# togheppi/pytorch-super-resolution-model-collection

Measured on AMD Instinct MI355X. Metric: ESPCN x4 LR->HR images/sec (infer), higher is better.
Workload: dtype f32 storage/accumulate; fp32-faithful products on the fp16 matrix cores: operands scaled by exact powers of two, split into two fp16 planes, 3 MFMAs per product (f16x3, ~3e-7 rms vs fp64, like fp32 MFMA); 1 GPU; c2: ESPCN x4 inference, 256x256 LR, batch 64 per GPU, fp32, random-init N(0,0.02); parallelism=replicas x1 (no collective)

## Files before the change

### pytorch_super_resolution_model_collection_amd/csrc/conv_pair.hip

```cpp
#include "conv_bfw.h"

namespace srk {

namespace {

constexpr int PR_TH = 8, PR_TW = 16, PR_HW = 18;
constexpr int PR_NSLOTPIX = 6 * PR_HW, PR_NPIXP = PR_NSLOTPIX + 2;
constexpr int PR_NKEEP = 2 * PR_HW, PR_KP = PR_NKEEP + 2;
constexpr int PR_XR = 14, PR_XC = 23, PR_XP = 24;
constexpr int PR_NSLOT = 3, PR_NKBUF = 3;
constexpr int PR_WL2 = 9 * 2 * 256;
constexpr int PR_HBUF = 4 * PR_NPIXP;
constexpr int PR_KBUF = 2 * 4 * PR_KP;
constexpr int PR_PLANE = PR_NSLOT * PR_HBUF + PR_NKBUF * PR_KBUF;
constexpr int PR_XBUF = 2 * PR_XR * PR_XP;
constexpr unsigned PR_AMAX_CAP = 1u << 14;
constexpr int PR_ARRIVE = 1, PR_DEPART = 2;
constexpr int PR_XLD = 24;
constexpr int PR_W1P = 2 * 2 * 4 * 2 * 64;
constexpr int PR_W1P_FLOATS = 144;
constexpr size_t PR_W1P_BYTES = (size_t)PR_W1P * 16 + PR_W1P_FLOATS * 4;
constexpr size_t PR_LDS = (size_t)PR_WL2 * 16 + (size_t)2 * PR_PLANE * 16 + (size_t)2 * PR_XBUF * 8 + 64;
static_assert(PR_LDS <= 160 * 1024, "k_espcn_pair: LDS");

__device__ unsigned g_pair_timeouts = 0;
__device__ unsigned g_pair_scans = 0;

typedef unsigned v4u_t __attribute__((ext_vector_type(4)));

struct PairParams {
  const float* x;
  const uint4* w1p;
  const float* b1;
  const uint4* wq2;
  const float* w2_descale;
  const float* b2;
  float* y;
  float* x_amax;
  float* y_amax;
  size_t xn;
  int amax_mode;
  int N, H, W, OH, OW, tiles_y, img_tiles, ntiles;
  unsigned x_img_bytes, y_bytes;
};

__device__ __forceinline__ float pr_slice_absmax(const float* __restrict__ x, size_t lo, size_t hi, size_t n, bool tail,
                                                 int t, int nt) {
  const f32x4* x4 = reinterpret_cast<const f32x4*>(x);
  float m = 0.f;
  for (size_t base = lo; base < hi; base += (size_t)nt * PR_XLD) {
    f32x4 v[PR_XLD];
#pragma unroll
    for (int k = 0; k < PR_XLD; ++k) {
      const size_t e = base + (size_t)t + (size_t)k * nt;
      v[k] = x4[e < hi ? e : hi - 1];
    }
#pragma unroll
    for (int k = 0; k < PR_XLD; ++k) m = abs_max4(m, v[k]);
  }
  if (tail) {
    const size_t e = (n & ~(size_t)3) + (size_t)t;
    if (t < 3 && e < n) m = fmaxf(m, fabsf(x[e]));
  }
  return m;
}

__global__ __launch_bounds__(128) void k_espcn_pair_prep(const float* __restrict__ w1, const float* __restrict__ b1,
                                                         uint4* __restrict__ out) {
  const int lane = threadIdx.x & 63, c1 = threadIdx.x >> 6;
  const int j = lane & 15, kq = lane >> 4;
  float wsum = 0.f, wmax = 0.f;
  {
    const float* wc = w1 + lane * 75;
    for (int i = 0; i < 75; ++i) {
      const float a = fabsf(wc[i]);
      wsum += a;
      wmax = fmaxf(wmax, a);
    }
  }
  const float wm = wave_max(wmax);
  const float sw1 = exp2i(amax_scale_exp(wm));
#pragma unroll
  for (int nf = 0; nf < 2; ++nf) {
    const int co = c1 * 32 + nf * 16 + j;
#pragma unroll
    for (int ks = 0; ks < 4; ++ks) {
      const int q = 4 * ks + kq, dy = q / 3, dx0 = 2 * (q - 3 * (q / 3));
      float f[8];
#pragma unroll
      for (int e = 0; e < 8; ++e) {
        const int dx = dx0 + (e >> 2), ci = e & 3;
        const bool on = q < 15 && ci < 3 && dx < 5;
        f[e] = on ? w1[((co * 3 + (on ? ci : 0)) * 5 + (on ? dy : 0)) * 5 + (on ? dx : 0)] : 0.f;
      }
      uint4 pl[2];
      split8h(f, sw1, pl);
      out[(((c1 * 2 + nf) * 4 + ks) * 2 + 0) * 64 + lane] = pl[0];
      out[(((c1 * 2 + nf) * 4 + ks) * 2 + 1) * 64 + lane] = pl[1];
    }
  }
  if (c1 == 0) {
    float* t = reinterpret_cast<float*>(out + PR_W1P);
    t[lane] = wsum;
    t[64 + lane] = fabsf(b1[lane]);
    if (lane == 0) t[128] = wm;
  }
}

__global__ __launch_bounds__(512, 1) void k_espcn_pair(PairParams B) {
  extern __shared__ __attribute__((aligned(16))) uint4 smem4[];
  uint4* wl2 = smem4;
  uint4* ring = smem4 + PR_WL2;
  uint4* keep = ring + PR_NSLOT * PR_HBUF;
  uint2* xin_all = reinterpret_cast<uint2*>(ring + 2 * PR_PLANE);
  lds_cnt_t* cnt = (lds_cnt_t*)(xin_all + 2 * PR_XBUF);
  const int tid = threadIdx.x, lane = tid & 63, wave = tid >> 6;
  const int grp = wave >> 2, gw = wave & 3, lt = tid & 255;
  const int j = lane & 15, kq = lane >> 4;
  uint2* xin = xin_all + grp * PR_XBUF;

  const float* w1t = reinterpret_cast<const float*>(B.w1p + PR_W1P);
  const int nblk = gridDim.x;
  float xmax = 0.f;
  if (tid < 14) cnt[tid] = 0u;
  if (B.amax_mode) {
    float* red = reinterpret_cast<float*>(xin_all);
    const size_t n4 = B.xn >> 2;
    const float m = wave_max(pr_slice_absmax(B.x, (size_t)blockIdx.x * n4 / nblk, (size_t)(blockIdx.x + 1) * n4 / nblk, B.xn,
                                             blockIdx.x == 0, tid, 512));
    if (lane == 0) red[wave] = m;
    __syncthreads();
    if (tid == 0) {
      float b = red[0];
#pragma unroll
      for (int i = 1; i < 8; ++i) b = fmaxf(b, red[i]);
      const unsigned was = atomicMax(reinterpret_cast<unsigned*>(B.x_amax + (blockIdx.x & 15) * 16), __float_as_uint(b));
      asm volatile("s_waitcnt vmcnt(0)" ::"v"(was) : "memory");
      __hip_atomic_fetch_add(reinterpret_cast<unsigned*>(B.x_amax) + PR_ARRIVE, 1u, __ATOMIC_RELAXED, __HIP_MEMORY_SCOPE_AGENT);
    }
  } else {
    xmax = amax_read(B.x_amax);
  }

  {
    static_assert(PR_WL2 == 9 * 512, "k_espcn_pair: filter copy");
    v4u_t wv[9];
#pragma unroll
    for (int i = 0; i < 9; ++i) wv[i] = *reinterpret_cast<const v4u_t*>(B.wq2 + tid + 512 * i);
#pragma unroll
    for (int i = 0; i < 9; ++i) *reinterpret_cast<v4u_t*>(wl2 + tid + 512 * i) = wv[i];
  }

  const int c1 = gw >> 1, mh = gw & 1;
  const int mhu = __builtin_amdgcn_readfirstlane(mh), rhu = __builtin_amdgcn_readfirstlane(gw >> 1);
  uint4 w1f[2][4][2];
#pragma unroll
  for (int nf = 0; nf < 2; ++nf)
#pragma unroll
    for (int ks = 0; ks < 4; ++ks)
#pragma unroll
      for (int pl = 0; pl < 2; ++pl) w1f[nf][ks][pl] = B.w1p[(((c1 * 2 + nf) * 4 + ks) * 2 + pl) * 64 + lane];
  const float wsum = w1t[lane], babs = w1t[64 + lane];
  int koff[4], mpix[5], moff[5], tpix[2], toff[2];
#pragma unroll
  for (int ks = 0; ks < 4; ++ks) {
    const int q = (4 * ks + kq) < 15 ? 4 * ks + kq : 14;
    koff[ks] = (q / 3) * PR_XP + 2 * (q - 3 * (q / 3));
  }
#pragma unroll
  for (int m = 0; m < 5; ++m) {
    mpix[m] = 16 * (m < 4 ? 4 * mh + m : 8) + j;
    const int p = PR_NKEEP + mpix[m];
    moff[m] = (p / PR_HW) * PR_XP + p % PR_HW;
  }
#pragma unroll
  for (int m = 0; m < 2; ++m) {
    tpix[m] = 16 * (2 * mh + m) + j;
    const int p = tpix[m] < PR_NKEEP ? tpix[m] : PR_NKEEP - 1;
    toff[m] = (p / PR_HW) * PR_XP + p % PR_HW;
  }
  const int wr_slot = (kq >> 1) * PR_NPIXP * 16 + (kq & 1) * 8, wr_keep = (c1 * 4 + (kq >> 1)) * PR_KP * 16 + (kq & 1) * 8;

  const int rh = gw >> 1, nf2 = gw & 1;
  const int pj = j < 4 ? 2 * j : (j < 12 ? 2 * j - 7 : 2 * j - 16);
  const int lane_b = (4 * rh - 2) * PR_HW + pj + kq * PR_NPIXP;
  const int lane_k = pj + kq * PR_KP;
  const int lane_a = kq * 32 + nf2 * 16 + j;
  float b2v[4];
#pragma unroll
  for (int e = 0; e < 4; ++e) b2v[e] = B.b2[nf2 * 16 + 4 * kq + e];

  const int xcd = blockIdx.x & 7;
  int first, count;
  {
    const int lb = xcd * (nblk >> 3) + (xcd < (nblk & 7) ? xcd : (nblk & 7)) + (blockIdx.x >> 3);
    const int per = B.ntiles / nblk, rem = B.ntiles - per * nblk;
    first = lb * per + (lb < rem ? lb : rem);
    count = per + (lb < rem ? 1 : 0);
  }
  count = __builtin_amdgcn_readfirstlane(count);

  const __amdgpu_buffer_rsrc_t yr = buffer_rsrc(B.y, B.y_bytes);
  const unsigned HW_ = (unsigned)(B.H * B.W);
  float xv[2][3];
  auto xload = [&](int i) {
    const bool valid = i < count;
    const int t = first + (valid ? i : 0);
    const int n = t / B.img_tiles, rem = t - n * B.img_tiles;
    const int tx = rem / B.tiles_y, ty = rem - tx * B.tiles_y;
    const __amdgpu_buffer_rsrc_t xr = buffer_rsrc(B.x + (size_t)n * 3 * HW_, B.x_img_bytes);
#pragma unroll
    for (int s = 0; s < 2; ++s) {
      const int q = lt + 256 * s, qy = q / PR_XC, qx = q - qy * PR_XC;
      const bool ok = valid && q < PR_XR * PR_XC;
      const unsigned o = ok ? 4u * (unsigned)((ty * PR_TH + qy) * B.W + tx * PR_TW + qx) : 0x80000000u;
#pragma unroll
      for (int c = 0; c < 3; ++c)
        xv[s][c] = __builtin_bit_cast(float, __builtin_amdgcn_raw_buffer_load_b32(xr, (int)(o + (ok ? 4u * c * HW_ : 0u)), 0, 0));
    }
  };
  auto l1_frags = [&](auto nm, const int* off, f32x4 (*a)[2]) {
    constexpr int NM = decltype(nm)::value;
#pragma unroll
    for (int m = 0; m < NM; ++m) a[m][0] = a[m][1] = (f32x4){0.f, 0.f, 0.f, 0.f};
#pragma unroll
    for (int ks = 0; ks < 4; ++ks) {
#pragma unroll
      for (int m = 0; m < NM; ++m) {
        const int pa = off[m] + koff[ks];
        const uint2 h0 = xin[pa], h1 = xin[pa + 1];
        const uint2 l0 = xin[PR_XR * PR_XP + pa], l1 = xin[PR_XR * PR_XP + pa + 1];
        const uint4 xh = make_uint4(h0.x, h0.y, h1.x, h1.y), xm = make_uint4(l0.x, l0.y, l1.x, l1.y);
#pragma unroll
        for (int nf = 0; nf < 2; ++nf) {
          a[m][nf] = mfma16h(w1f[nf][ks][0], xm, a[m][nf]);
          a[m][nf] = mfma16h(w1f[nf][ks][1], xh, a[m][nf]);
          a[m][nf] = mfma16h(w1f[nf][ks][0], xh, a[m][nf]);
        }
      }
    }
  };
  bool dead = false;
  float amax = 0.f;
  xload(grp);
  if (B.amax_mode && wave == 0) {
    unsigned* ctr = reinterpret_cast<unsigned*>(B.x_amax);
    bool late = B.amax_mode == 2;
    if (!late) {
      unsigned spins = 0;
      while ((int)((unsigned)__builtin_amdgcn_readfirstlane((int)__hip_atomic_load(ctr + PR_ARRIVE, __ATOMIC_RELAXED,
                                                                                   __HIP_MEMORY_SCOPE_AGENT)) -
                   (unsigned)nblk) < 0) {
        __builtin_amdgcn_s_sleep(16);
        if (++spins > PR_AMAX_CAP) {
          late = true;
          break;
        }
      }
    }
    asm volatile("" ::: "memory");
    const float sv = wave_max(__hip_atomic_load(B.x_amax + (lane & 15) * 16, __ATOMIC_RELAXED, __HIP_MEMORY_SCOPE_AGENT));
    if (lane == 0) {
      cnt[14] = __float_as_uint(sv);
      cnt[15] = late ? 1u : 0u;
      const unsigned d = __hip_atomic_fetch_add(ctr + PR_DEPART, 1u, __ATOMIC_RELAXED, __HIP_MEMORY_SCOPE_AGENT);
      if (d + 1u == (unsigned)nblk) {
        __hip_atomic_store(ctr + PR_ARRIVE, 0u, __ATOMIC_RELAXED, __HIP_MEMORY_SCOPE_AGENT);
        __hip_atomic_store(ctr + PR_DEPART, 0u, __ATOMIC_RELAXED, __HIP_MEMORY_SCOPE_AGENT);
      }
    }
  }
  __syncthreads();
  if (B.amax_mode) {
    xmax = __uint_as_float(lds_cnt_peek(cnt + 14));
    if (lds_cnt_peek(cnt + 15)) {
      float* red = reinterpret_cast<float*>(xin_all);
      const float m = wave_max(pr_slice_absmax(B.x, 0, B.xn >> 2, B.xn, true, tid, 512));
      if (lane == 0) red[wave] = m;
      __syncthreads();
#pragma unroll
      for (int i = 0; i < 8; ++i) xmax = fmaxf(xmax, red[i]);
      xmax = __uint_as_float((unsigned)__builtin_amdgcn_readfirstlane((int)__float_as_uint(xmax)));
      __syncthreads();
      if (tid == 0) atomicAdd(&g_pair_scans, 1u);
    }
  }
  const int kx = amax_scale_exp(xmax);
  const float bnd = wave_max(fabsf(babs) + wsum * xmax);
  const int kw1 = amax_scale_exp(w1t[128]);
  const int km = amax_scale_exp(bnd);
  const float sx1 = exp2i(kx), sxm = exp2i(km);
  const float dsc1 = exp2i(-kx) * exp2i(-kw1);
  const float dsc2 = exp2i(-km) * B.w2_descale[0];

  unsigned own = 0;
  unsigned kseq = 0;
  int typrev = 0;
  for (int i = grp; i < count; i += 2, ++own) {
    const int t = first + i;
    const int n = t / B.img_tiles, rem = t - n * B.img_tiles;
    const int tx = rem / B.tiles_y, ty = rem - tx * B.tiles_y;
    const bool fresh = i == 0 || ty == 0;
    const bool hand = i + 1 < count && ty + 1 < B.tiles_y;
    kseq = i == grp ? (grp == 0 ? 1u : 2u + (ty == 0 ? 1u : 0u))
                    : kseq + 2u + (typrev + 1 == B.tiles_y ? 1u : 0u) + (ty == 0 ? 1u : 0u);
    typrev = ty;
    const unsigned kb = kseq % PR_NKBUF, ku = kseq / PR_NKBUF, tb = (kseq - 1u) % PR_NKBUF, tu = (kseq - 1u) / PR_NKBUF;
#pragma unroll
    for (int s = 0; s < 2; ++s) {
      const int q = lt + 256 * s;
      if (q < PR_XR * PR_XC) {
        const int qy = q / PR_XC, qx = q - qy * PR_XC;
        unsigned h01, m01, h2, m2;
        split2h(xv[s][0], xv[s][1], sx1, h01, m01);
        split2h(xv[s][2], 0.f, sx1, h2, m2);
        xin[qy * PR_XP + qx] = make_uint2(h01, h2);
        xin[PR_XR * PR_XP + qy * PR_XP + qx] = make_uint2(m01, m2);
      }
    }
    lds_cnt_signal(cnt + 6 + grp);
    xload(i + 2);
    lds_cnt_wait(cnt + 6 + grp, 4u * (own + 1), dead);

    float b1v[2][4];
#pragma unroll
    for (int nf = 0; nf < 2; ++nf)
#pragma unroll
      for (int e = 0; e < 4; ++e) b1v[nf][e] = B.b1[c1 * 32 + nf * 16 + 4 * kq + e];
    auto l1_store = [&](const f32x4 (&a)[2], unsigned char* base, int pix, int pitch) {
#pragma unroll
      for (int nf = 0; nf < 2; ++nf) {
        float v[4];
#pragma unroll
        for (int e = 0; e < 4; ++e) v[e] = fmaxf(__builtin_fmaf(a[nf][e], dsc1, b1v[nf][e]), 0.f);
        unsigned h01, m01, h23, m23;
        split2h(v[0], v[1], sxm, h01, m01);
        split2h(v[2], v[3], sxm, h23, m23);
        *reinterpret_cast<uint2*>(base + ((2 * nf) * pitch + pix) * 16) = make_uint2(h01, h23);
        *reinterpret_cast<uint2*>(base + (PR_PLANE + (2 * nf) * pitch + pix) * 16) = make_uint2(m01, m23);
      }
    };
    auto l1_tile = [&](auto nm) {
      constexpr int NM = decltype(nm)::value;
      f32x4 a1[NM][2];
      l1_frags(nm, moff, a1);
      const unsigned st = 2u * (unsigned)i + c1, slot = st % PR_NSLOT, use = st / PR_NSLOT;
      unsigned char* hb = reinterpret_cast<unsigned char*>(ring + slot * PR_HBUF) + wr_slot;
      lds_cnt_wait(cnt + 3 + slot, 4u * use, dead);
#pragma unroll
      for (int m = 0; m < NM; ++m)
        if (mpix[m] < PR_NSLOTPIX) l1_store(a1[m], hb, mpix[m], PR_NPIXP);
      lds_cnt_signal(cnt + slot);
      unsigned char* kp = reinterpret_cast<unsigned char*>(keep + kb * PR_KBUF) + wr_keep;
      lds_cnt_wait(cnt + 11 + kb, 8u * ku, dead);
#pragma unroll
      for (int m = 2; m < NM; ++m)
        if (mpix[m] >= PR_NSLOTPIX) l1_store(a1[m], kp, mpix[m] - PR_NSLOTPIX, PR_KP);
      lds_cnt_signal(cnt + 8 + kb);
    };
    const int vr = B.OH - ty * PR_TH;
    if (mhu == 1 && vr <= 3) {
      const unsigned st = 2u * (unsigned)i + c1, slot = st % PR_NSLOT, use = st / PR_NSLOT;
      lds_cnt_wait(cnt + 3 + slot, 4u * use, dead);
      lds_cnt_signal(cnt + slot);
      lds_cnt_wait(cnt + 11 + kb, 8u * ku, dead);
      lds_cnt_signal(cnt + 8 + kb);
    } else if (mh == (int)(own & 1)) {
      l1_tile(std::integral_constant<int, 5>{});
    } else {
      l1_tile(std::integral_constant<int, 4>{});
    }
    if (fresh) {
      f32x4 at[2][2];
      l1_frags(std::integral_constant<int, 2>{}, toff, at);
      unsigned char* kp = reinterpret_cast<unsigned char*>(keep + tb * PR_KBUF) + wr_keep;
      lds_cnt_wait(cnt + 11 + tb, 8u * tu, dead);
#pragma unroll
      for (int m = 0; m < 2; ++m)
        if (tpix[m] < PR_NKEEP) l1_store(at[m], kp, tpix[m], PR_KP);
      lds_cnt_signal(cnt + 8 + tb);
    }

    lds_cnt_wait(cnt + 8 + (rh == 0 ? tb : kb), 4u * ((rh == 0 ? tu : ku) + 1u), dead);
    if (rhu == 1 && vr <= 4) {
#pragma unroll
      for (int cc = 0; cc < 2; ++cc) {
        const unsigned st = 2u * (unsigned)i + cc, slot = st % PR_NSLOT, use = st / PR_NSLOT;
        lds_cnt_wait(cnt + slot, 2u * (use + 1), dead);
        lds_cnt_signal(cnt + 3 + slot);
      }
      lds_cnt_signal(cnt + 11 + tb, fresh ? 2u : 1u);
      lds_cnt_signal(cnt + 11 + kb, hand ? 1u : 2u);
    } else {
      f32x4 acc[4];
#pragma unroll
      for (int r = 0; r < 4; ++r) acc[r] = (f32x4){0.f, 0.f, 0.f, 0.f};
#pragma unroll
      for (int cc = 0; cc < 2; ++cc) {
        const unsigned st = 2u * (unsigned)i + cc, slot = st % PR_NSLOT, use = st / PR_NSLOT;
        lds_cnt_wait(cnt + slot, 2u * (use + 1), dead);
        const uint4* hb = ring + slot * PR_HBUF + lane_b;
        const uint4* kr = keep + (rh == 0 ? tb : kb) * PR_KBUF + cc * 4 * PR_KP + lane_k - (rh == 0 ? 0 : 4 * PR_HW);
        const uint4* pa = rh == 0 ? kr : hb;
        const uint4* pc = rh == 0 ? hb : kr;
#pragma unroll
        for (int v = 0; v < 3; ++v) {
          uint4 fa[3][2];
#pragma unroll
          for (int u = 0; u < 3; ++u) {
            fa[u][0] = wl2[((u * 3 + v) * 2 + cc) * 256 + lane_a];
            fa[u][1] = wl2[((u * 3 + v) * 2 + cc) * 256 + 128 + lane_a];
          }
#pragma unroll
          for (int R = 0; R < 6; ++R) {
            const uint4* px = R < 2 ? pa : (R < 4 ? hb : pc);
            const uint4 xh = px[R * PR_HW + v], xm = px[R * PR_HW + v + PR_PLANE];
#pragma unroll
            for (int u = 0; u < 3; ++u) {
              const int r = R - u;
              if (r >= 0 && r < 4) {
                acc[r] = mfma16h(fa[u][0], xm, acc[r]);
                acc[r] = mfma16h(fa[u][1], xh, acc[r]);
                acc[r] = mfma16h(fa[u][0], xh, acc[r]);
              }
            }
          }
        }
        lds_cnt_signal(cnt + 3 + slot);
      }
      lds_cnt_signal(cnt + 11 + tb, fresh ? 2u : 1u);
      lds_cnt_signal(cnt + 11 + kb, hand ? 1u : 2u);
      const int oc = tx * PR_TW + pj;
#pragma unroll
      for (int r = 0; r < 4; ++r) {
        const int orow = ty * PR_TH + 4 * rh + r;
        const bool ok = oc < B.OW && orow < B.OH;
        f32x4 v;
#pragma unroll
        for (int e = 0; e < 4; ++e) v[e] = fmaxf(__builtin_fmaf(acc[r][e], dsc2, b2v[e]), 0.f);
        if (ok) amax = fmaxf(amax, fmaxf(fmaxf(v[0], v[1]), fmaxf(v[2], v[3])));
        const unsigned o = ok ? 4u * (unsigned)(((n * B.OH + orow) * B.OW + oc) * 32 + nf2 * 16 + 4 * kq) : 0x80000000u;
        __builtin_amdgcn_raw_buffer_store_b128(__builtin_bit_cast(v4u_t, v), yr, (int)o, 0, 0);
      }
    }
  }
  if (B.y_amax) amax_commit(B.y_amax, amax, blockIdx.x + wave, amax_peek(B.y_amax, blockIdx.x + wave));
  if (dead && lane == 0) atomicAdd(&g_pair_timeouts, 1u);
}

}

int espcn_pair_launch(int N, int H, int W, const float* x, const void* w1p, const float* b1, const void* wp2,
                      const float* b2, float* y, float* x_amax, int amax_mode, float* y_amax, bool force, hipStream_t s) {
  if (N < 1 || H < 7 || W < 7 || !x_amax) return -1;
  const int OH = H - 6, OW = W - 6;
  const int tiles_y = (OH + PR_TH - 1) / PR_TH, tiles_x = (OW + PR_TW - 1) / PR_TW;
  const long ntiles = (long)N * tiles_y * tiles_x;
  const size_t x_img = (size_t)3 * H * W * 4, y_bytes = (size_t)N * OH * OW * 32 * 4;
  if (ntiles >= (1L << 29) || x_img >= (1ull << 31) || y_bytes >= (1ull << 31)) return -1;
  if (!force) {
    if ((double)OH * OW < 0.85 * (double)tiles_y * tiles_x * (PR_TH * PR_TW)) return -1;
    if (ntiles < 4L * kNumCU) return -1;
  }
  const size_t elems = (size_t)9 * 64 * 32;
  const char* prepared = reinterpret_cast<const char*>(wp2) + bf3_prepared_offset(elems);
  const char* fsec = prepared + f16_section_offset(64, 32, 9);
  PairParams B{};
  B.x = x; B.w1p = reinterpret_cast<const uint4*>(w1p); B.b1 = b1; B.b2 = b2; B.y = y; B.x_amax = x_amax; B.y_amax = y_amax;
  B.xn = (size_t)N * 3 * H * W;
  B.amax_mode = amax_mode;
  B.wq2 = reinterpret_cast<const uint4*>(fsec);
  B.w2_descale = reinterpret_cast<const float*>(fsec + bf3_main_bytes(64, 32, 9));
  B.N = N; B.H = H; B.W = W; B.OH = OH; B.OW = OW; B.tiles_y = tiles_y; B.img_tiles = tiles_x * tiles_y;
  B.ntiles = (int)ntiles;
  B.x_img_bytes = (unsigned)x_img;
  B.y_bytes = (unsigned)y_bytes;
  int grid = kNumCU;
  if (grid > ntiles) grid = (int)ntiles;
  note_amax_written(y_amax != nullptr);
  note_kernel("k_espcn_pair");
  launch_lds<&k_espcn_pair>(dim3(grid), dim3(512), PR_LDS, s, B);
  return check_launch("espcn_pair");
}

int pair_ring_timeouts(int reset) {
  unsigned v = 0;
  if (hipMemcpyFromSymbol(&v, HIP_SYMBOL(g_pair_timeouts), sizeof(v)) != hipSuccess) {
    (void)hipGetLastError();
    return -1;
  }
  if (reset && v) {
    const unsigned z = 0;
    (void)hipMemcpyToSymbol(HIP_SYMBOL(g_pair_timeouts), &z, sizeof(z));
  }
  return (int)v;
}

int pair_scans(int reset) {
  unsigned v = 0;
  if (hipMemcpyFromSymbol(&v, HIP_SYMBOL(g_pair_scans), sizeof(v)) != hipSuccess) {
    (void)hipGetLastError();
    return -1;
  }
  if (reset && v) {
    const unsigned z = 0;
    (void)hipMemcpyToSymbol(HIP_SYMBOL(g_pair_scans), &z, sizeof(z));
  }
  return (int)v;
}

int espcn_pair_prepare(const float* w1, const float* b1, void* out, hipStream_t s) {
  hipLaunchKernelGGL(k_espcn_pair_prep, dim3(1), dim3(128), 0, s, w1, b1, reinterpret_cast<uint4*>(out));
  return check_launch("espcn_pair_prepare");
}
size_t espcn_pair_prepared_bytes() { return PR_W1P_BYTES; }

}

extern "C" size_t srk_espcn_pair_prepared_bytes(void) { return srk::espcn_pair_prepared_bytes(); }

extern "C" int srk_espcn_pair_prepare(const float* w1, const float* b1, void* w1_prepared, void* stream) {
  SRK_REQUIRE(w1 && b1 && w1_prepared, "espcn_pair_prepare: null pointer");
  SRK_REQUIRE((uintptr_t)w1_prepared % 16 == 0, "espcn_pair_prepare: w1_prepared must be 16-byte aligned");
  return srk::espcn_pair_prepare(w1, b1, w1_prepared, (hipStream_t)stream);
}

extern "C" int srk_espcn_pair_scans(int reset) { return srk::pair_scans(reset); }

extern "C" int srk_espcn_pair_forward(int N, int H, int W, const float* x, const void* w1_prepared, const float* b1,
                                      const float* w2_packed_fwd, const float* b2, float* y, float* x_amax,
                                      int x_amax_compute, float* y_amax, int force, void* stream) {
  if (!x || !w1_prepared || !b1 || !w2_packed_fwd || !b2 || !y || !x_amax) return SRK_ERR_UNSUPPORTED;
  if (((uintptr_t)x | (uintptr_t)y | (uintptr_t)w1_prepared) % 16 != 0) return SRK_ERR_UNSUPPORTED;
  const int mode = x_amax_compute ? ((force & 2) ? 2 : 1) : 0;
  const int rc = srk::espcn_pair_launch(N, H, W, x, w1_prepared, b1, w2_packed_fwd, b2, y, x_amax, mode, y_amax,
                                        (force & 1) != 0, (hipStream_t)stream);
  return rc == -1 ? SRK_ERR_UNSUPPORTED : rc;
}
```

Measured before the change: 74320 images/s.

## Repack conv1 input and weights to fold fp16 split products into fewer MFMAs

Reorganizes the first conv layer's K dimension so that the hi/lo fp16 planes of the input and weights are packed into the same 8-element K slot. One MFMA per k-group then computes the cross terms, replacing three MFMAs over four k-steps with one MFMA over eight k-steps. The input tile in LDS becomes a 16-byte-per-pixel interleaved layout plus a transposed row buffer for the leftover taps, and pixels within the MFMA tile are permuted. This adds zero-initialisation of the input buffers and more complex addressing, and it risks changing the numerical equivalence of the split-fp16 scheme.

```diff
diff --git a/pytorch_super_resolution_model_collection_amd/csrc/conv_pair.hip b/pytorch_super_resolution_model_collection_amd/csrc/conv_pair.hip
--- a/pytorch_super_resolution_model_collection_amd/csrc/conv_pair.hip
+++ b/pytorch_super_resolution_model_collection_amd/csrc/conv_pair.hip
@@ -13,14 +13,17 @@
 constexpr int PR_HBUF = 4 * PR_NPIXP;
 constexpr int PR_KBUF = 2 * 4 * PR_KP;
 constexpr int PR_PLANE = PR_NSLOT * PR_HBUF + PR_NKBUF * PR_KBUF;
-constexpr int PR_XBUF = 2 * PR_XR * PR_XP;
+constexpr int PR_XPQ = PR_XR * PR_XP * 16;
+constexpr int PR_XT = PR_XPQ + 32;
+constexpr int PR_XBUF = PR_XT + PR_XR * PR_XP * 8;
+constexpr unsigned long long PR_FPIX = 0xfdb9eca875316420ull;
 constexpr unsigned PR_AMAX_CAP = 1u << 14;
 constexpr int PR_ARRIVE = 1, PR_DEPART = 2;
 constexpr int PR_XLD = 24;
-constexpr int PR_W1P = 2 * 2 * 4 * 2 * 64;
+constexpr int PR_W1P = 2 * 2 * 8 * 64;
 constexpr int PR_W1P_FLOATS = 144;
 constexpr size_t PR_W1P_BYTES = (size_t)PR_W1P * 16 + PR_W1P_FLOATS * 4;
-constexpr size_t PR_LDS = (size_t)PR_WL2 * 16 + (size_t)2 * PR_PLANE * 16 + (size_t)2 * PR_XBUF * 8 + 64;
+constexpr size_t PR_LDS = (size_t)PR_WL2 * 16 + (size_t)2 * PR_PLANE * 16 + (size_t)2 * PR_XBUF + 64;
 static_assert(PR_LDS <= 160 * 1024, "k_espcn_pair: LDS");
 
 __device__ unsigned g_pair_timeouts = 0;
@@ -65,6 +68,17 @@
   return m;
 }
 
+enum { PR_KTAP, PR_KROW, PR_KNONE };
+struct PrKGroup {
+  int kind, dy, dx;
+};
+__device__ __forceinline__ constexpr PrKGroup pr_kgroup(int ks, int kq) {
+  if (ks < 5) return {PR_KTAP, ks, kq};
+  if (ks == 5) return {PR_KTAP, (kq >> 1) + 2 * (kq & 1), 4};
+  if (ks == 6) return kq == 0 ? PrKGroup{PR_KTAP, 4, 4} : (kq == 1 ? PrKGroup{PR_KNONE, 0, 0} : PrKGroup{PR_KROW, 2 * kq - 4, 0});
+  return kq == 3 ? PrKGroup{PR_KNONE, 0, 0} : PrKGroup{PR_KROW, kq == 2 ? 4 : 2 * kq + 1, 0};
+}
+
 __global__ __launch_bounds__(128) void k_espcn_pair_prep(const float* __restrict__ w1, const float* __restrict__ b1,
                                                          uint4* __restrict__ out) {
   const int lane = threadIdx.x & 63, c1 = threadIdx.x >> 6;
@@ -84,19 +98,19 @@
   for (int nf = 0; nf < 2; ++nf) {
     const int co = c1 * 32 + nf * 16 + j;
 #pragma unroll
-    for (int ks = 0; ks < 4; ++ks) {
-      const int q = 4 * ks + kq, dy = q / 3, dx0 = 2 * (q - 3 * (q / 3));
+    for (int ks = 0; ks < 8; ++ks) {
+      const PrKGroup g = pr_kgroup(ks, kq);
       float f[8];
 #pragma unroll
       for (int e = 0; e < 8; ++e) {
-        const int dx = dx0 + (e >> 2), ci = e & 3;
-        const bool on = q < 15 && ci < 3 && dx < 5;
-        f[e] = on ? w1[((co * 3 + (on ? ci : 0)) * 5 + (on ? dy : 0)) * 5 + (on ? dx : 0)] : 0.f;
+        const bool tap = g.kind == PR_KTAP;
+        const bool on = tap || (g.kind == PR_KROW && e < 5);
+        const int ci = tap ? (e < 6 ? e % 3 : e - 6) : 2, dx = tap ? g.dx : (e < 5 ? e : 0);
+        f[e] = on ? w1[((co * 3 + ci) * 5 + g.dy) * 5 + dx] : 0.f;
       }
       uint4 pl[2];
       split8h(f, sw1, pl);
-      out[(((c1 * 2 + nf) * 4 + ks) * 2 + 0) * 64 + lane] = pl[0];
-      out[(((c1 * 2 + nf) * 4 + ks) * 2 + 1) * 64 + lane] = pl[1];
+      out[((c1 * 2 + nf) * 8 + ks) * 64 + lane] = g.kind == PR_KTAP ? make_uint4(pl[0].x, pl[0].y, pl[0].z, pl[1].w) : pl[1];
     }
   }
   if (c1 == 0) {
@@ -112,12 +126,12 @@
   uint4* wl2 = smem4;
   uint4* ring = smem4 + PR_WL2;
   uint4* keep = ring + PR_NSLOT * PR_HBUF;
-  uint2* xin_all = reinterpret_cast<uint2*>(ring + 2 * PR_PLANE);
+  unsigned char* xin_all = reinterpret_cast<unsigned char*>(ring + 2 * PR_PLANE);
   lds_cnt_t* cnt = (lds_cnt_t*)(xin_all + 2 * PR_XBUF);
   const int tid = threadIdx.x, lane = tid & 63, wave = tid >> 6;
   const int grp = wave >> 2, gw = wave & 3, lt = tid & 255;
   const int j = lane & 15, kq = lane >> 4;
-  uint2* xin = xin_all + grp * PR_XBUF;
+  unsigned char* xin = xin_all + grp * PR_XBUF;
 
   const float* w1t = reinterpret_cast<const float*>(B.w1p + PR_W1P);
   const int nblk = gridDim.x;
@@ -153,31 +167,35 @@
 
   const int c1 = gw >> 1, mh = gw & 1;
   const int mhu = __builtin_amdgcn_readfirstlane(mh), rhu = __builtin_amdgcn_readfirstlane(gw >> 1);
-  uint4 w1f[2][4][2];
+  uint4 w1f[2][8];
 #pragma unroll
   for (int nf = 0; nf < 2; ++nf)
 #pragma unroll
-    for (int ks = 0; ks < 4; ++ks)
-#pragma unroll
-      for (int pl = 0; pl < 2; ++pl) w1f[nf][ks][pl] = B.w1p[(((c1 * 2 + nf) * 4 + ks) * 2 + pl) * 64 + lane];
+    for (int ks = 0; ks < 8; ++ks) w1f[nf][ks] = B.w1p[((c1 * 2 + nf) * 8 + ks) * 64 + lane];
   const float wsum = w1t[lane], babs = w1t[64 + lane];
-  int koff[4], mpix[5], moff[5], tpix[2], toff[2];
-#pragma unroll
-  for (int ks = 0; ks < 4; ++ks) {
-    const int q = (4 * ks + kq) < 15 ? 4 * ks + kq : 14;
-    koff[ks] = (q / 3) * PR_XP + 2 * (q - 3 * (q / 3));
-  }
+  const int jp = (int)((PR_FPIX >> (4 * j)) & 15);
+  int mpix[5], moff[5], tpix[2], toff[2];
 #pragma unroll
   for (int m = 0; m < 5; ++m) {
-    mpix[m] = 16 * (m < 4 ? 4 * mh + m : 8) + j;
+    mpix[m] = 16 * (m < 4 ? 4 * mh + m : 8) + jp;
     const int p = PR_NKEEP + mpix[m];
-    moff[m] = (p / PR_HW) * PR_XP + p % PR_HW;
+    moff[m] = (p / PR_HW) * PR_XP + p % PR_HW + kq;
   }
 #pragma unroll
   for (int m = 0; m < 2; ++m) {
-    tpix[m] = 16 * (2 * mh + m) + j;
+    tpix[m] = 16 * (2 * mh + m) + jp;
     const int p = tpix[m] < PR_NKEEP ? tpix[m] : PR_NKEEP - 1;
-    toff[m] = (p / PR_HW) * PR_XP + p % PR_HW;
+    toff[m] = (p / PR_HW) * PR_XP + p % PR_HW + kq;
+  }
+  const int k5 = pr_kgroup(5, kq).dy * PR_XP + 4 - kq;
+  int kmul[2], kadd[2], kd[2];
+#pragma unroll
+  for (int s = 0; s < 2; ++s) {
+    const PrKGroup own = pr_kgroup(6 + s, kq), g = own.kind == PR_KNONE ? pr_kgroup(6 + s, kq - 1) : own;
+    kmul[s] = g.kind == PR_KTAP ? 16 : 8;
+    kd[s] = g.kind == PR_KTAP ? 8 : 32;
+    asm volatile("" : "+v"(kd[s]));
+    kadd[s] = g.kind == PR_KTAP ? 16 * (g.dy * PR_XP + g.dx - kq) : PR_XT + 8 * (g.dy * PR_XP - kq);
   }
   const int wr_slot = (kq >> 1) * PR_NPIXP * 16 + (kq & 1) * 8, wr_keep = (c1 * 4 + (kq >> 1)) * PR_KP * 16 + (kq & 1) * 8;
 
@@ -224,19 +242,19 @@
 #pragma unroll
     for (int m = 0; m < NM; ++m) a[m][0] = a[m][1] = (f32x4){0.f, 0.f, 0.f, 0.f};
 #pragma unroll
-    for (int ks = 0; ks < 4; ++ks) {
+    for (int ks = 0; ks < 8; ++ks) {
 #pragma unroll
       for (int m = 0; m < NM; ++m) {
-        const int pa = off[m] + koff[ks];
-        const uint2 h0 = xin[pa], h1 = xin[pa + 1];
-        const uint2 l0 = xin[PR_XR * PR_XP + pa], l1 = xin[PR_XR * PR_XP + pa + 1];
-        const uint4 xh = make_uint4(h0.x, h0.y, h1.x, h1.y), xm = make_uint4(l0.x, l0.y, l1.x, l1.y);
-#pragma unroll
-        for (int nf = 0; nf < 2; ++nf) {
-          a[m][nf] = mfma16h(w1f[nf][ks][0], xm, a[m][nf]);
-          a[m][nf] = mfma16h(w1f[nf][ks][1], xh, a[m][nf]);
-          a[m][nf] = mfma16h(w1f[nf][ks][0], xh, a[m][nf]);
+        uint4 xc;
+        if (ks < 6) {
+          xc = *reinterpret_cast<const uint4*>(xin + 16 * (off[m] + (ks < 5 ? ks * PR_XP : k5)));
+        } else {
+          const int pa = __mul24(off[m], kmul[ks & 1]) + kadd[ks & 1];
+          const uint2 ca = *reinterpret_cast<const uint2*>(xin + pa), cb = *reinterpret_cast<const uint2*>(xin + pa + kd[ks & 1]);
+          xc = make_uint4(ca.x, ca.y, cb.x, cb.y);
         }
+#pragma unroll
+        for (int nf = 0; nf < 2; ++nf) a[m][nf] = mfma16h(w1f[nf][ks], xc, a[m][nf]);
       }
     }
   };
@@ -285,6 +303,8 @@
       if (tid == 0) atomicAdd(&g_pair_scans, 1u);
     }
   }
+  for (int i = tid; i < 2 * PR_XBUF / 16; i += 512) reinterpret_cast<uint4*>(xin_all)[i] = make_uint4(0u, 0u, 0u, 0u);
+  __syncthreads();
   const int kx = amax_scale_exp(xmax);
   const float bnd = wave_max(fabsf(babs) + wsum * xmax);
   const int kw1 = amax_scale_exp(w1t[128]);
@@ -314,8 +334,10 @@
         unsigned h01, m01, h2, m2;
         split2h(xv[s][0], xv[s][1], sx1, h01, m01);
         split2h(xv[s][2], 0.f, sx1, h2, m2);
-        xin[qy * PR_XP + qx] = make_uint2(h01, h2);
-        xin[PR_XR * PR_XP + qy * PR_XP + qx] = make_uint2(m01, m2);
+        *reinterpret_cast<uint4*>(xin + 16 * (qy * PR_XP + qx)) = make_uint4(h01, h2 | (m01 << 16), (m01 >> 16) | (m2 << 16), h01);
+        unsigned short* tq = reinterpret_cast<unsigned short*>(xin + PR_XT) + 4 * (qy * PR_XP + qx);
+#pragma unroll
+        for (int k = 0; k < 4; ++k) tq[-3 * k] = (unsigned short)h2;
       }
     }
     lds_cnt_signal(cnt + 6 + grp);
```

After: 77420 images/s (median of 6 runs). 1.04x the previous value.
